# sethdford/csm-mlx

Hardware: AMD Instinct MI355X
Metric: audio frames/sec (24 kHz) csm_1b greedy, 10 s utterances, 1/2/4/8 GPU (higher is better)
Workload: dtype bf16; 1 GPU; csm_1b greedy generate(), 10 s utterances (125 frames) + Mimi decode; top_k=0, stream=False, context_segments=0, model=csm_1b (synthetic seed-0 weights), global_batch=1, per_gpu_batch=1, frames=125, mimi_decode=True, parallelism=dp1

## Files before the change

### csm-mlx_amd/csrc/bb_step.hip

```cpp
#include <type_traits>

#include "csm_kernels.h"
#include "handoff.h"

namespace {

using namespace handoff;

constexpr int NWG = BB_STEP_WGS, NT = BB_STEP_THREADS;
constexpr int D = 2048, F = 8192, HQ = 32, HKV = 8, HD = 64, NL = BB_STEP_LAYERS;
constexpr int QKV = (HQ + 2 * HKV) * HD;
constexpr int NATT = HQ;

constexpr int REP = 4;
constexpr size_t G_QKV = 0;
constexpr size_t G_ATT = G_QKV + 2 * QKV;
constexpr size_t G_X = G_ATT + 2 * REP * rs_of(D);
constexpr size_t G_PART = G_X + 2 * REP * rs_of(D);
constexpr size_t G_TOTAL = G_PART + (size_t)2 * NWG * D;

struct Lds {
  float x[D];
  float xn[D];
  float att[D];
  float red[8][NWG];
  float wsum[8][8];
  float sq[8];
  alignas(16) float hb[32];
  float2 rope[HD / 2];
  float q[HD], kn[HD], vn[HD];
  float am[8], al[8], ao[8][HD];
  float Ks[128][HD + 4], Vs[128][HD];
  alignas(16) float xq[D / 32][36];
  float xh[D / 32];
  alignas(16) float aq[D / 32][36];
  float ah[D / 32];
};

struct Ctx : HandoffCtx<BbStepArgs, Lds, REP> {
  __device__ void stamp(int slot) const {
    if (p.stamps && tid == 0 && slot < BB_STEP_STAMPS) p.stamps[(size_t)w * BB_STEP_STAMPS + slot] = __builtin_amdgcn_s_memrealtime();
  }
};

constexpr int PROBE_DELAY = 32;
constexpr int DELAY_E2 = PROBE_DELAY;

template <int GPT, int DELAY = PROBE_DELAY>
__device__ __forceinline__ void gather(Ctx& c, const u64* buf, int n, float* out) {
  const unsigned tag = c.tag();
  u64 g[GPT];
  __builtin_amdgcn_s_sleep(DELAY);
#pragma unroll
  for (int u = 0; u < GPT; ++u) {
    const int i = c.tid + u * NT;
    g[u] = i < n ? gload(buf + i) : ((u64)tag << 32);
  }
  for (unsigned spin = 0;; ++spin) {
    bool ok = true;
#pragma unroll
    for (int u = 0; u < GPT; ++u) ok &= (unsigned)(g[u] >> 32) == tag;
    if (ok || spin_fail(c, spin)) break;
    __builtin_amdgcn_s_sleep(1);
#pragma unroll
    for (int u = 0; u < GPT; ++u) {
      const int i = c.tid + u * NT;
      if (i < n && (unsigned)(g[u] >> 32) != tag) g[u] = gload(buf + i);
    }
  }
  c.stamp(c.e + 1);
#pragma unroll
  for (int u = 0; u < GPT; ++u) {
    const int i = c.tid + u * NT;
    if (i < n) out[i] = __uint_as_float((unsigned)g[u]);
  }
  __syncthreads();
}

__device__ __forceinline__ int el(const Ctx& c, int j) { return (j >> 1) * (D / 2) + 2 * c.tid + (j & 1); }
struct Nw { float v[D / NT]; };
__device__ __forceinline__ Nw nw_fetch(const Ctx& c, const float* nw) {
  Nw r;
#pragma unroll
  for (int j = 0; j < D / NT; ++j) r.v[j] = nw[el(c, j)];
  return r;
}
__device__ __forceinline__ void rms(Ctx& c, const Nw& nw, float* out) {
  if (c.wave == 0) {
    float s = 0.f;
#pragma unroll 8
    for (int k = c.lane; k < D; k += 64) s = fmaf(c.L.x[k], c.L.x[k], s);
    s = wave_sum(s);
    if (c.lane == 0) c.L.wsum[0][0] = s;
  }
  __syncthreads();
  const float r = rsqrtf(c.L.wsum[0][0] / (float)D + c.p.eps);
#pragma unroll
  for (int j = 0; j < D / NT; ++j) out[el(c, j)] = c.L.x[el(c, j)] * r * nw.v[j];
  __syncthreads();
}

__device__ __forceinline__ void gather_x(Ctx& c, const u64* buf, const Nw& nw) {
  constexpr int GPT = D / NT;
  const unsigned tag = c.tag();
  float sq = 0.f;
  const int poff[GPT / 2] = {2 * c.tid, D / 2 + 2 * c.tid};
  poll_pairs<GPT / 2, PROBE_DELAY, 1>(buf, 0x7fffffff, poff, tag, [&](unsigned spin) { return spin_fail(c, spin); },
                                      [&](const u32x4_t (&g)[GPT / 2]) {
#pragma unroll
    for (int h = 0; h < GPT / 2; ++h) {
      const float v0 = __uint_as_float(g[h].x), v1 = __uint_as_float(g[h].z);
      *reinterpret_cast<float2*>(&c.L.x[poff[h]]) = make_float2(v0, v1);
      *reinterpret_cast<float2*>(&c.L.xn[poff[h]]) = make_float2(v0 * nw.v[2 * h], v1 * nw.v[2 * h + 1]);
      sq = fmaf(v0, v0, sq);
      sq = fmaf(v1, v1, sq);
    }
  });
  c.stamp(c.e + 1);
  sq = wave_sum(sq);
  if (c.lane == 0) c.L.sq[c.wave] = sq;
  __syncthreads();
}
__device__ __forceinline__ float row_rs(const Ctx& c) {
  float s = c.L.sq[0];
#pragma unroll
  for (int w = 1; w < 8; ++w) s += c.L.sq[w];
  return rsqrtf(s / (float)D + c.p.eps);
}

struct WQ { u32x4_t a[6]; };
struct WO { u32x4_t a[4]; };
struct WMq { u32x4_t g[2][4]; u32x4_t d[4]; };

__device__ __forceinline__ void load_q(Ctx& c, int l, WQ& r) {
  const bf16_t* base = c.p.wqkv[l] + (size_t)(12 * c.w + 6 * (c.tid >> 8)) * D;
  const int v = (c.tid & 255) * 16;
#pragma unroll
  for (int i = 0; i < 6; ++i) r.a[i] = bload<2>(base, v, i * D * 2);
}
__device__ __forceinline__ void load_o(Ctx& c, int l, WO& r) {
  const bf16_t* base = c.p.wo[l] + (size_t)(8 * c.w + 4 * (c.tid >> 8)) * D;
  const int v = (c.tid & 255) * 16;
#pragma unroll
  for (int i = 0; i < 4; ++i) r.a[i] = bload<2>(base, v, i * D * 2);
}
__device__ __forceinline__ void load_mq(Ctx& c, int l, int Q, WMq& r) {
  const bf16_t* g = c.p.wgu[l] + (size_t)(64 * c.w + 16 * Q + 2 * c.wave) * D;
#pragma unroll
  for (int i = 0; i < 2; ++i)
#pragma unroll
    for (int j = 0; j < 4; ++j) r.g[i][j] = bload<2>(g, c.lane * 16, i * D * 2 + j * 64 * 16);
  const bf16_t* d = c.p.wdc[l] + (size_t)(4 * c.w + Q) * D * 8;
#pragma unroll
  for (int k = 0; k < 4; ++k)
    r.d[k] = bload<2>(d, c.tid * 16, k * NT * 8 * 2);
}

template <int R>
__device__ __forceinline__ void rows_reduce(Ctx& c, float (&s)[R]) {
#pragma unroll
  for (int i = 0; i < R; ++i) s[i] = wave_sum(s[i]);
  if (c.lane == 0) {
#pragma unroll
    for (int i = 0; i < R; ++i) c.L.wsum[c.wave][i] = s[i];
  }
  __syncthreads();
}
__device__ __forceinline__ float row_total(const Ctx& c, int h, int i) {
  return ((c.L.wsum[4 * h][i] + c.L.wsum[4 * h + 1][i]) + c.L.wsum[4 * h + 2][i]) + c.L.wsum[4 * h + 3][i];
}

__device__ __forceinline__ void phase_qkv(Ctx& c, int l, int pos, const WQ& W, bool sc) {
  float s[6];
  const float* xc = c.L.xn + 8 * (c.tid & 255);
#pragma unroll
  for (int i = 0; i < 6; ++i) s[i] = dot8(W.a[i], xc);
  rows_reduce<6>(c, s);
  if (c.tid < 6) {
    const int h = c.tid / 3, i0 = 2 * (c.tid % 3), n = 12 * c.w + 6 * h + i0;
    float a = row_total(c, h, i0), b = row_total(c, h, i0 + 1);
    if (sc) {
      const float rs = row_rs(c);
      a *= rs;
      b *= rs;
    }
    if (n < (HQ + HKV) * HD) {
      const float2 cs = c.L.rope[(n % HD) / 2];
      const float y0 = a * cs.x - b * cs.y, y1 = b * cs.x + a * cs.y;
      a = y0;
      b = y1;
    }
    u64* g = c.buf(G_QKV, QKV);
    gput(g + n, a, c.tag());
    gput(g + n + 1, b, c.tag());
    if (n >= HQ * HD) {
      const int nn = n < (HQ + HKV) * HD ? n - HQ * HD : n - (HQ + HKV) * HD;
      float* cache = n < (HQ + HKV) * HD ? c.p.kc[l] : c.p.vc[l];
      *reinterpret_cast<float2*>(cache + ((size_t)(nn / HD) * c.p.S_cap + pos) * HD + nn % HD) = make_float2(a, b);
    }
  }
}

struct KvPass { float4 kv[4], vv[4]; };

__device__ __forceinline__ void kv_pass_load(const Ctx& c, const float* K, const float* V, int pos, int k0, KvPass& kp) {
#pragma unroll
  for (int u = 0; u < 4; ++u) {
    const int idx = c.tid + NT * u, r = idx >> 4, c4 = idx & 15, j = k0 + r;
    const float4* ks = reinterpret_cast<const float4*>(j < pos ? K + (size_t)j * HD : c.L.kn);
    const float4* vs = reinterpret_cast<const float4*>(j < pos ? V + (size_t)j * HD : c.L.vn);
    kp.kv[u] = j <= pos ? ks[c4] : make_float4(0.f, 0.f, 0.f, 0.f);
    kp.vv[u] = j <= pos ? vs[c4] : make_float4(0.f, 0.f, 0.f, 0.f);
  }
}

__device__ __forceinline__ void attn_begin(Ctx& c, int l, int pos, KvPass& kp) {
  const int a = c.w, g = a / (HQ / HKV);
  {
    const u64* buf = c.p.gbuf + G_QKV + (size_t)((c.e - 1) & 1) * QKV;
    const unsigned tag = c.tag() - 1u;
    if (c.tid < 3 * HD) {
      const int part = c.tid / HD, d = c.tid % HD;
      const int idx = part == 0 ? a * HD + d : (part == 1 ? HQ * HD + g * HD + d : (HQ + HKV) * HD + g * HD + d);
      __builtin_amdgcn_s_sleep(PROBE_DELAY);
      u64 v = gload(buf + idx);
      for (unsigned spin = 0; (unsigned)(v >> 32) != tag; ++spin) {
        if (spin_fail(c, spin)) break;
        __builtin_amdgcn_s_sleep(1);
        v = gload(buf + idx);
      }
      const float f = __uint_as_float((unsigned)v);
      if (part == 0) c.L.q[d] = f * 0.125f;
      else if (part == 1) c.L.kn[d] = f;
      else c.L.vn[d] = f;
    }
    __syncthreads();
    c.stamp(c.e);
  }
// ... 15 lines not shown
      *reinterpret_cast<float4*>(&c.L.Ks[r][4 * c4]) = kp.kv[u];
      *reinterpret_cast<float4*>(&c.L.Vs[r][4 * c4]) = kp.vv[u];
    }
    __syncthreads();
    const int blk = c.wave - ((k0 >> 6) & 7);
    if (blk == 0 || blk == 1) {
      const int b0 = k0 + 64 * blk;
      if (b0 < n) {
        const int j = b0 + c.lane;
        const float4* kr = reinterpret_cast<const float4*>(c.L.Ks[64 * blk + c.lane]);
        const float4* q4 = reinterpret_cast<const float4*>(c.L.q);
        float d0 = 0.f, d1 = 0.f, d2 = 0.f, d3 = 0.f;
#pragma unroll
        for (int d4 = 0; d4 < HD / 4; ++d4) {
          const float4 qq = q4[d4], kk = kr[d4];
          d0 = fmaf(qq.x, kk.x, d0);
          d1 = fmaf(qq.y, kk.y, d1);
          d2 = fmaf(qq.z, kk.z, d2);
          d3 = fmaf(qq.w, kk.w, d3);
        }
        const float sc = j <= pos ? (d0 + d1) + (d2 + d3) : -INFINITY;
        const float m_new = fmaxf(m_run, wave_max(sc));
        const float alpha = m_run == -INFINITY ? 0.f : expf(m_run - m_new);
        const float pj = j <= pos ? expf(sc - m_new) : 0.f;
        l_run = l_run * alpha + wave_sum(pj);
        o *= alpha;
        const int pji = __float_as_int(pj);
#pragma unroll
        for (int u = 0; u < 64; ++u)
          o = fmaf(__int_as_float(__builtin_amdgcn_readlane(pji, u)), c.L.Vs[64 * blk + u][c.lane], o);
        m_run = m_new;
      }
    }
  }
  c.L.ao[c.wave][c.lane] = o;
  if (c.lane == 0) { c.L.am[c.wave] = m_run; c.L.al[c.wave] = l_run; }
  __syncthreads();
  if (c.wave < REP) {
    float M = -INFINITY;
#pragma unroll
    for (int v = 0; v < 8; ++v) M = fmaxf(M, c.L.am[v]);
    float Ls = 0.f, O = 0.f;
#pragma unroll
    for (int v = 0; v < 8; ++v) {
      const float wv = c.L.am[v] == -INFINITY ? 0.f : expf(c.L.am[v] - M);
      Ls = fmaf(c.L.al[v], wv, Ls);
      O = fmaf(c.L.ao[v][c.lane], wv, O);
    }
    c.put(G_ATT, D, a * HD + c.lane, O / Ls, c.wave);
  }
}

__device__ __forceinline__ void phase_o(Ctx& c, const WO& W) {
  float s[4];
  const float* xc = c.L.att + 8 * (c.tid & 255);
#pragma unroll
  for (int i = 0; i < 4; ++i) s[i] = dot8(W.a[i], xc);
  rows_reduce<4>(c, s);
  if (c.tid < 8 * REP) {
    const int q = c.tid / REP, h = q / 4, i = q % 4, n = 8 * c.w + q;
    c.put(G_X, D, n, c.L.x[n] + row_total(c, h, i), c.tid % REP);
  }
}

template <int Q>
__device__ __forceinline__ void phase_mq(Ctx& c, const WMq& m, float (&acc)[4], float rs) {
  float t[2];
#pragma unroll
  for (int i = 0; i < 2; ++i) {
    float s = dot8(m.g[i][0], c.L.xn + 8 * c.lane);
#pragma unroll
    for (int j = 1; j < 4; ++j) s += dot8(m.g[i][j], c.L.xn + 8 * (c.lane + 64 * j));
    t[i] = wave_sum(s);
  }
  if (c.lane == 0) c.L.hb[8 * Q + c.wave] = silu_f(rs * t[0]) * (rs * t[1]);
  __syncthreads();
#pragma unroll
  for (int k = 0; k < 4; ++k) {
    const float v = dot8(m.d[k], c.L.hb + 8 * Q);
    acc[k] = Q == 0 ? v : acc[k] + v;
  }
}

__device__ __forceinline__ void phase_reduce(Ctx& c) {
  const unsigned tag = c.tag();
  const u64* g = c.buf(G_PART, (size_t)NWG * D);
  const int v = c.tid >> 1, half = c.tid & 1;
  const int poff[2] = {v * D + 8 * c.w + 4 * half, v * D + 8 * c.w + 4 * half + 2};
  poll_pairs<2, PROBE_DELAY, 1>(g, 0x7fffffff, poff, tag, [&](unsigned spin) { return spin_fail(c, spin); },
                                [&](const u32x4_t (&q)[2]) {
#pragma unroll
    for (int h = 0; h < 2; ++h) {
      c.L.red[4 * half + 2 * h][v] = __uint_as_float(q[h].x);
      c.L.red[4 * half + 2 * h + 1][v] = __uint_as_float(q[h].z);
    }
  });
  c.stamp(c.e + 1);
  __syncthreads();
  ++c.e;
  {
    const float* r = c.L.red[c.wave];
    float s = ((r[4 * c.lane] + r[4 * c.lane + 1]) + r[4 * c.lane + 2]) + r[4 * c.lane + 3];
    s = wave_sum(s);
    if (c.lane < REP) {
      const int n = 8 * c.w + c.wave;
      c.put(G_X, D, n, c.L.x[n] + s, c.lane);
    }
  }
}

struct WQ4 { u32x4_t a[2]; unsigned s[2]; };
struct WO4 { u32x4_t a; unsigned s; };
struct WM4 { u32x4_t g[8]; unsigned gs[8]; u32x4_t d[4]; unsigned ds[4]; };
constexpr int RB = D / 2, SBR = D / 64 * 4;
constexpr int SB_QKV = QKV * RB, SB_O = D * RB, SB_GU = 2 * F * RB, SB_DN = D * F / 2;

__device__ __forceinline__ void load_q4(Ctx& c, int l, WQ4& r) {
  const char* W = reinterpret_cast<const char*>(c.p.wqkv[l]);
  const int r0 = 12 * c.w, va = c.wave * RB + c.lane * 16, vb = (8 + (c.wave & 3)) * RB + c.lane * 16;
  r.a[0] = bload<2>(W, va, r0 * RB);
  r.a[1] = bload<2>(W, vb, r0 * RB);
  const int sa = c.wave * SBR + (c.lane >> 1) * 4, sb = (8 + (c.wave & 3)) * SBR + (c.lane >> 1) * 4;
  r.s[0] = bload4(W, sa, SB_QKV + r0 * SBR);
  r.s[1] = bload4(W, sb, SB_QKV + r0 * SBR);
}
__device__ __forceinline__ void load_o4(Ctx& c, int l, WO4& r) {
  const char* W = reinterpret_cast<const char*>(c.p.wo[l]);
  r.a = bload<2>(W, c.wave * RB + c.lane * 16, 8 * c.w * RB);
  r.s = bload4(W, c.wave * SBR + (c.lane >> 1) * 4, SB_O + 8 * c.w * SBR);
}
__device__ __forceinline__ void load_m4(Ctx& c, int l, WM4& r) {
  const char* G = reinterpret_cast<const char*>(c.p.wgu[l]);
  const int r0 = 64 * c.w + 8 * c.wave;
#pragma unroll
  for (int i = 0; i < 8; ++i) {
    r.g[i] = bload<2>(G, 8 * c.wave * RB + c.lane * 16, (64 * c.w + i) * RB);
    r.gs[i] = bload4(G, 8 * c.wave * SBR + (c.lane >> 1) * 4, SB_GU + (64 * c.w + i) * SBR);
  }
  (void)r0;
  const char* Dn = reinterpret_cast<const char*>(c.p.wdc[l]);
#pragma unroll
  for (int k = 0; k < 4; ++k) {
    r.d[k] = bload<2>(Dn, c.tid * 16, (c.w * D + k * NT) * 16);
    r.ds[k] = bload4(Dn, c.tid * 4, SB_DN + ((c.w >> 1) * D + k * NT) * 4);
  }
}

__device__ __forceinline__ void half_group_sums(Ctx& c, const float (&pair)[2], float* out) {
#pragma unroll
  for (int h = 0; h < 2; ++h) {
    const float v = sum16(pair[h]);
    if ((c.tid & 15) == 0) out[(h * (D / 2) + 2 * c.tid) >> 5] = v;
  }
}
__device__ __forceinline__ void gather_x4(Ctx& c, const u64* buf, const Nw& nw) {
  const int poff[2] = {2 * c.tid, D / 2 + 2 * c.tid};
  float sq = 0.f, pr[2];
  poll_pairs<2, PROBE_DELAY, 1>(buf, 0x7fffffff, poff, c.tag(), [&](unsigned spin) { return spin_fail(c, spin); },
                                [&](const u32x4_t (&g)[2]) {
#pragma unroll
    for (int h = 0; h < 2; ++h) {
      const float v0 = __uint_as_float(g[h].x), v1 = __uint_as_float(g[h].z);
      const float a = v0 * nw.v[2 * h], b = v1 * nw.v[2 * h + 1];
      *reinterpret_cast<float2*>(&c.L.x[poff[h]]) = make_float2(v0, v1);
      *reinterpret_cast<float2*>(&c.L.xq[0][0] + q4p(poff[h])) = make_float2(a, b);
      sq = fmaf(v0, v0, sq);
// ... 89 lines not shown
  if (c.lane < 4) {
    const float gt = rs * (c.lane == 0 ? t[0] : (c.lane == 1 ? t[2] : (c.lane == 2 ? t[4] : t[6])));
    const float up = rs * (c.lane == 0 ? t[1] : (c.lane == 1 ? t[3] : (c.lane == 2 ? t[5] : t[7])));
    c.L.hb[4 * c.wave + c.lane] = silu_f(gt) * up;
  }
  __syncthreads();
  float hsum = 0.f;
#pragma unroll
  for (int j = 0; j < 32; j += 4) {
    const float4 v = *reinterpret_cast<const float4*>(&c.L.hb[j]);
    hsum += (v.x + v.y) + (v.z + v.w);
  }
#pragma unroll
  for (int k = 0; k < 4; ++k) acc[k] = q4dot32(W.d[k], c.L.hb, W.ds[k], hsum);
}

}

__global__ __launch_bounds__(NT, 1) void bb_step_q4_kernel(BbStepArgs p) {
  __shared__ __attribute__((aligned(16))) Lds L;
  Ctx c{{p, L, (int)blockIdx.x, (int)threadIdx.x, (int)(threadIdx.x & 63), (int)(threadIdx.x >> 6), 0u, 0}};
  c.tag0 = __hip_atomic_load(p.epoch, __ATOMIC_RELAXED, __HIP_MEMORY_SCOPE_AGENT) + 1u;
  c.stamp(0);
  const int pos = p.pos[0];
  WQ4 wq;
  WO4 wo;
  WM4 wm;
  load_q4(c, 0, wq);
  Nw nw1 = nw_fetch(c, p.n1[0]);
  for (int k = c.tid; k < D; k += NT) L.x[k] = p.x[k];
  if (c.tid < HD / 2) L.rope[c.tid] = reinterpret_cast<const float2*>(p.rope)[(size_t)pos * (HD / 2) + c.tid];
  __syncthreads();
  stage_x4(c, nw1);
  for (int l = 0; l < NL; ++l) {
    c.refresh();
    phase_qkv4(c, l, pos, wq);
    ++c.e;
    const bool attn_wg = c.w < NATT;
    if (!attn_wg) {
      load_o4(c, l, wo);
      load_m4(c, l, wm);
    }
    const Nw nw2 = nw_fetch(c, p.n2[l]);
    if (attn_wg) {
      KvPass kp;
      attn_begin(c, l, pos, kp);
      attn_rest(c, l, pos, kp);
      load_o4(c, l, wo);
      load_m4(c, l, wm);
    }
    if (attn_wg) gather_att4(c, c.rbuf(G_ATT, D));
    else gather_att4<DELAY_E2>(c, c.rbuf(G_ATT, D));
    ++c.e;
    c.refresh();
    phase_o4(c, wo);
    if (l + 1 < NL) load_q4(c, l + 1, wq);
    gather_x4(c, c.rbuf(G_X, D), nw2);
    const float rs2 = row_rs(c);
    ++c.e;
    c.refresh();
    float acc[4];
    phase_m4(c, wm, acc, rs2);
    {
      u64* g = c.buf(G_PART, (size_t)NWG * D) + (size_t)c.w * D;
#pragma unroll
      for (int k = 0; k < 4; ++k) gput(g + c.tid + NT * k, acc[k], c.tag());
    }
    nw1 = nw_fetch(c, l + 1 < NL ? p.n1[l + 1] : p.norm);
    c.refresh();
    phase_reduce(c);
    gather_x4(c, c.rbuf(G_X, D), nw1);
    ++c.e;
  }
  c.refresh();
  if (c.w == 0) {
    const float rs = row_rs(c);
    for (int k = c.tid; k < D; k += NT) p.h_last[k] = (&L.xq[0][0])[q4p(k)] * rs;
  }
  c.stamp(BB_STEP_STAMPS - 1);
  if (c.w == 0 && c.tid == 0) __hip_atomic_store(p.epoch, c.tag0 - 1u + (unsigned)c.e, __ATOMIC_RELAXED, __HIP_MEMORY_SCOPE_AGENT);
}

namespace {
}

__global__ __launch_bounds__(NT, 1) void bb_step_kernel(BbStepArgs p) {
  __shared__ __attribute__((aligned(16))) Lds L;
  Ctx c{{p, L, (int)blockIdx.x, (int)threadIdx.x, (int)(threadIdx.x & 63), (int)(threadIdx.x >> 6), 0u, 0}};
  c.tag0 = __hip_atomic_load(p.epoch, __ATOMIC_RELAXED, __HIP_MEMORY_SCOPE_AGENT) + 1u;
  c.stamp(0);
  const int pos = p.pos[0];
  WQ wq;
  WO wo;
  WMq mq[4];
  load_q(c, 0, wq);
  Nw nw1 = nw_fetch(c, p.n1[0]);
  for (int k = c.tid; k < D; k += NT) L.x[k] = p.x[k];
  if (c.tid < HD / 2) L.rope[c.tid] = reinterpret_cast<const float2*>(p.rope)[(size_t)pos * (HD / 2) + c.tid];
  __syncthreads();
  for (int l = 0; l < NL; ++l) {
    c.refresh();
    const bool fold1 = l > 0;
    if (!fold1) rms(c, nw1, L.xn);
    phase_qkv(c, l, pos, wq, fold1);
    ++c.e;
    const bool attn_wg = c.w < NATT;
    KvPass kp;
    load_o(c, l, wo);
    load_mq(c, l, 0, mq[0]);
    if (!attn_wg) {
      load_mq(c, l, 1, mq[1]);
      load_mq(c, l, 2, mq[2]);
    }
    const Nw nw2 = nw_fetch(c, p.n2[l]);
    if (attn_wg) {
      attn_begin(c, l, pos, kp);
      attn_rest(c, l, pos, kp);
      load_mq(c, l, 1, mq[1]);
    }
    if (attn_wg) gather<D / NT>(c, c.rbuf(G_ATT, D), D, L.att);
    else gather<D / NT, DELAY_E2>(c, c.rbuf(G_ATT, D), D, L.att);
    ++c.e;
    c.refresh();
    phase_o(c, wo);
    if (l + 1 < NL) load_q(c, l + 1, wq);
    gather_x(c, c.rbuf(G_X, D), nw2);
    const float rs2 = row_rs(c);
    ++c.e;
    c.refresh();
    float acc[4];
    phase_mq<0>(c, mq[0], acc, rs2);
    if (attn_wg) load_mq(c, l, 2, mq[2]);
    phase_mq<1>(c, mq[1], acc, rs2);
    load_mq(c, l, 3, mq[3]);
    phase_mq<2>(c, mq[2], acc, rs2);
    phase_mq<3>(c, mq[3], acc, rs2);
    {
      u64* g = c.buf(G_PART, (size_t)NWG * D) + (size_t)c.w * D;
#pragma unroll
      for (int k = 0; k < 4; ++k) gput(g + c.tid + NT * k, acc[k], c.tag());
    }
    nw1 = nw_fetch(c, l + 1 < NL ? p.n1[l + 1] : p.norm);
    c.refresh();
    phase_reduce(c);
    gather_x(c, c.rbuf(G_X, D), nw1);
    ++c.e;
  }
  c.refresh();
  if (c.w == 0) {
    const float rs = row_rs(c);
    for (int k = c.tid; k < D; k += NT) p.h_last[k] = L.xn[k] * rs;
  }
  c.stamp(BB_STEP_STAMPS - 1);
  if (c.w == 0 && c.tid == 0) __hip_atomic_store(p.epoch, c.tag0 - 1u + (unsigned)c.e, __ATOMIC_RELAXED, __HIP_MEMORY_SCOPE_AGENT);
}

size_t bb_step_gbuf_bytes() { return G_TOTAL * sizeof(u64); }

void launch_bb_step(const BbStepArgs& p, hipStream_t st, bool q4) {
  if (q4) hipLaunchKernelGGL(bb_step_q4_kernel, dim3(NWG), dim3(NT), 0, st, p);
  else hipLaunchKernelGGL(bb_step_kernel, dim3(NWG), dim3(NT), 0, st, p);
}

const void* bb_step_kernel_ptr(bool q4) {
  return q4 ? reinterpret_cast<const void*>(&bb_step_q4_kernel) : reinterpret_cast<const void*>(&bb_step_kernel);
}
```

### csm-mlx_amd/csrc/csm_engine_weights.hip

```cpp
#include "csm_engine.h"

namespace {

void alloc_stack(csm_engine* e, Stack& s, const csm_llama_dims& d, int S_cap, const char* prefix) {
  s.d = d;
  s.S_cap = S_cap;
  s.L.resize(d.n_layers);
  const size_t D = d.hidden, F = d.intermediate, hd = d.head_dim;
  for (int i = 0; i < d.n_layers; ++i) {
    LayerW& l = s.L[i];
    l.wqkv = e->alloc(e->wbytes(s.qkv_rows(), D));
    l.wo = e->alloc(e->wbytes(D, s.q_dim()));
    l.wgu = e->alloc(e->wbytes(2 * F, D));
    l.wd = e->alloc(e->wbytes(D, F));
    if (e->wdt == WDT_BF16 && wdc_chunk((int)D) && F % wdc_chunk((int)D) == 0) l.wdc = e->alloc(D * F * 2);
    l.n1 = (float*)e->alloc(D * 4);
    l.n2 = (float*)e->alloc(D * 4);
    const std::string p = std::string(prefix) + ".layers." + std::to_string(i);
    for (const char* n : {".self_attn.q_proj.weight", ".self_attn.k_proj.weight", ".self_attn.v_proj.weight",
                          ".self_attn.o_proj.weight", ".mlp.gate_proj.weight", ".mlp.up_proj.weight",
                          ".mlp.down_proj.weight", ".input_layernorm.weight", ".post_attention_layernorm.weight"})
      e->required.push_back(p + n);
  }
  s.norm = (float*)e->alloc(D * 4);
  s.rope = (float*)e->alloc((size_t)S_cap * hd * 4);
  e->required.push_back(std::string(prefix) + ".norm.weight");
}

}

void ensure_batch(csm_engine* e, int B) {
  if (B <= e->B_max && !e->batch_allocs.empty()) return;
  HIPCHK(hipDeviceSynchronize());
  for (void* p : e->batch_allocs) (void)hipFree(p);
  e->batch_allocs.clear();
  if (e->g_body) { (void)hipGraphExecDestroy(e->g_body); e->g_body = nullptr; }
  if (e->g_head) { (void)hipGraphExecDestroy(e->g_head); e->g_head = nullptr; }
  e->g_B = -1;
  e->B_max = std::max(B, e->B_max);
  const size_t Bm = e->B_max, D = e->D, Dd = e->Dd, K = e->K, Vp = e->Vpad;
  for (Stack* s : {&e->bb, &e->dec}) {
    const size_t kv = Bm * s->d.n_kv_heads * (size_t)s->S_cap * s->d.head_dim * 4;
    for (LayerW& l : s->L) {
      l.kc = (float*)e->balloc(kv);
      l.vc = (float*)e->balloc(kv);
    }
  }
  e->h_last = (float*)e->balloc(Bm * D * 4);
  e->c0_logits = (float*)e->balloc(Bm * Vp * 4);
  e->force = (int*)e->balloc(Bm * K * 4);
  e->force_ce = (float*)e->balloc(Bm * K * 4);
  e->ci_logits = (float*)e->balloc((K - 1) * Bm * Vp * 4);
  e->dx = (float*)e->balloc(2 * Bm * Dd * 4);
  e->din = (float*)e->balloc(2 * Bm * D * 4);
  e->dq = (float*)e->balloc(2 * Bm * e->dec.q_dim() * 4);
  e->datt = (float*)e->balloc(2 * Bm * e->dec.q_dim() * 4);
  e->dmlp = (float*)e->balloc(2 * Bm * (size_t)e->dec.d.intermediate * 4);
  e->codes = (int*)e->balloc(Bm * K * 4);
  e->hist = (int*)e->balloc((size_t)e->F_cap * Bm * K * 4);
  e->pos = (int*)e->balloc(Bm * 4);
  e->n_frames = (int*)e->balloc(Bm * 4);
  e->done = (uint8_t*)e->balloc(Bm);
  e->seeds = (uint64_t*)e->balloc(Bm * 8);
  e->part_stride = (int)(Vp / 2);
  e->part = (unsigned long long*)e->balloc(K * Bm * (size_t)e->part_stride * 8);
  for (Stack* s : {&e->bb, &e->dec}) {
    const int Dm = s->d.hidden, F = s->d.intermediate, rows = (s == &e->bb) ? std::max(e->M_cap, (int)Bm) : 2 * (int)Bm;
    gemm_reserve(e->ws, s->qkv_rows(), Dm, rows);
    gemm_reserve(e->ws, Dm, s->q_dim(), rows);
    gemm_reserve(e->ws, 2 * F, Dm, rows);
    gemm_reserve(e->ws, Dm, F, rows);
  }
  gemm_reserve(e->ws, (int)Dd, (int)D, 2 * (int)Bm);
  gemm_reserve(e->ws, (int)Vp, (int)D, (int)Bm);
  gemm_reserve(e->ws, (int)Vp, (int)Dd, (int)Bm);
  {
    const int xm = GEMM_XS_MAX_M, rows = std::min(2 * (int)Bm, xm);
    size_t bD = 0, bA = 0, bF = 0;
    for (Stack* s : {&e->bb, &e->dec}) {
      const int Dm = s->d.hidden, F = s->d.intermediate;
      bD = std::max(bD, xs::bytes(xm, Dm));
      bA = std::max(bA, xs::bytes(xm, s->q_dim()));
// ... 297 lines not shown
  }
  CSM_CATCH
}

int csm_engine_destroy(csm_engine* e) {
  CSM_TRY { delete e; }
  CSM_CATCH
}

int csm_set_rope_table(csm_engine* e, int which, const float* table, int n_pos, int head_dim) {
  CSM_TRY {
    Stack& s = which == 0 ? e->bb : e->dec;
    if (head_dim != s.d.head_dim || n_pos < s.S_cap) throw CsmError(CSM_ERR_ARG, "rope table shape mismatch");
    HIPCHK(hipSetDevice(e->dev));
    HIPCHK(hipMemcpy(s.rope, table, (size_t)s.S_cap * head_dim * 4, hipMemcpyHostToDevice));
  }
  CSM_CATCH
}

int csm_load_tensor(csm_engine* e, const char* cname, const void* host, int src_dtype, const int64_t* shape,
                    int ndim) {
  CSM_TRY {
    HIPCHK(hipSetDevice(e->dev));
    const std::string name(cname);
    std::vector<int64_t> shp(shape, shape + ndim);
    auto numel = [&]() { int64_t n = 1; for (auto s : shp) n *= s; return (size_t)n; };
    auto expect = [&](std::initializer_list<int64_t> want) {
      if (shp != std::vector<int64_t>(want)) throw CsmError(CSM_ERR_ARG, "shape mismatch for " + name);
    };
    if (name.rfind("decoder.layers.0.", 0) == 0) e->proj_tab_dirty = true;
    e->tiled_dirty = true;
    if (e->wdt == WDT_Q4 && load_q4(e, name, host, src_dtype, shp)) return CSM_OK;
    if (src_dtype == CSM_U32) throw CsmError(CSM_ERR_ARG, "packed int4 tensor " + name + " needs a CSM_Q4 engine");
    const size_t es = e->wsz;
    auto conv = [&](size_t n) { return convert_to(host, src_dtype, n, e->wdt); };
    auto conv_f32 = [&](size_t n) { return convert_to(host, src_dtype, n, WDT_F32); };

    for (int which = 0; which < 2; ++which) {
      Stack& s = which == 0 ? e->bb : e->dec;
      const std::string pre = which == 0 ? "backbone." : "decoder.";
      if (name.rfind(pre, 0) != 0) continue;
      const int D = s.d.hidden, F = s.d.intermediate, hd = s.d.head_dim;
      const int qd = s.q_dim(), kvd = s.d.n_kv_heads * hd;
      if (name == pre + "norm.weight") {
        expect({D});
        auto h = conv_f32(D);
        HIPCHK(hipMemcpy(s.norm, h.data(), D * 4, hipMemcpyHostToDevice));
        e->loaded.insert(name);
        return CSM_OK;
      }
      int li = -1;
      char tail[128] = {0};
      if (sscanf(name.c_str() + pre.size(), "layers.%d.%127s", &li, tail) != 2 || li < 0 || li >= s.d.n_layers)
        throw CsmError(CSM_ERR_ARG, "unknown tensor " + name);
      LayerW& l = s.L[li];
      const std::string t(tail);
      if (t == "self_attn.q_proj.weight") {
        expect({qd, D});
        auto h = conv(numel());
        HIPCHK(hipMemcpy(l.wqkv, h.data(), h.size(), hipMemcpyHostToDevice));
      } else if (t == "self_attn.k_proj.weight" || t == "self_attn.v_proj.weight") {
        expect({kvd, D});
        auto h = conv(numel());
        const size_t row0 = qd + (t[10] == 'k' ? 0 : kvd);
        HIPCHK(hipMemcpy((char*)l.wqkv + row0 * D * es, h.data(), h.size(), hipMemcpyHostToDevice));
      } else if (t == "self_attn.o_proj.weight") {
        expect({D, qd});
        auto h = conv(numel());
        HIPCHK(hipMemcpy(l.wo, h.data(), h.size(), hipMemcpyHostToDevice));
      } else if (t == "mlp.gate_proj.weight" || t == "mlp.up_proj.weight") {
        expect({F, D});
        auto h = conv(numel());
        const size_t off = (t[4] == 'g') ? 0 : 1;
        HIPCHK(hipMemcpy2D((char*)l.wgu + off * D * es, 2 * D * es, h.data(), D * es, D * es, F,
                           hipMemcpyHostToDevice));
      } else if (t == "mlp.down_proj.weight") {
        expect({D, F});
        auto h = conv(numel());
        HIPCHK(hipMemcpy(l.wd, h.data(), h.size(), hipMemcpyHostToDevice));
        if (l.wdc) {
          const int R = wdc_chunk(D);
          const uint16_t* src = reinterpret_cast<const uint16_t*>(h.data());
          std::vector<uint16_t> t2((size_t)D * F);
          for (int c = 0; c < F / R; ++c)
            for (int n = 0; n < D; ++n)
              memcpy(&t2[((size_t)c * D + n) * R], src + (size_t)n * F + (size_t)c * R, R * 2);
          HIPCHK(hipMemcpy(l.wdc, t2.data(), t2.size() * 2, hipMemcpyHostToDevice));
        }
      } else if (t == "input_layernorm.weight" || t == "post_attention_layernorm.weight") {
        expect({D});
        auto h = conv_f32(D);
        HIPCHK(hipMemcpy(t[0] == 'i' ? l.n1 : l.n2, h.data(), D * 4, hipMemcpyHostToDevice));
      } else {
        throw CsmError(CSM_ERR_ARG, "unknown tensor " + name);
      }
      e->loaded.insert(name);
      return CSM_OK;
    }
    const int64_t D = e->D, Dd = e->Dd, V = e->V, K = e->K, Vp = e->Vpad;
    if (name == "text_embeddings.weight") {
      expect({e->dims.n_text_vocab, D});
      auto h = conv(numel());
      HIPCHK(hipMemcpy(e->text_emb, h.data(), h.size(), hipMemcpyHostToDevice));
    } else if (name == "audio_embeddings.weight") {
      e->proj_tab_dirty = true;
      expect({V * K, D});
      auto h = conv(numel());
      HIPCHK(hipMemcpy(e->audio_emb, h.data(), h.size(), hipMemcpyHostToDevice));
    } else if (name == "projection.weight") {
      e->proj_tab_dirty = true;
      expect({Dd, D});
      auto h = conv(numel());
      HIPCHK(hipMemcpy(e->proj, h.data(), h.size(), hipMemcpyHostToDevice));
    } else if (name == "codebook0_head.weight") {
      expect({V, D});
      auto h = conv(numel());
      HIPCHK(hipMemcpy(e->c0_head, h.data(), h.size(), hipMemcpyHostToDevice));
    } else if (name == "audio_head") {
      expect({K - 1, Dd, V});
      auto f = conv_f32(numel());
      const float* src = reinterpret_cast<const float*>(f.data());
      std::vector<float> t((size_t)(K - 1) * Vp * Dd, 0.f);
      for (int64_t c = 0; c < K - 1; ++c)
        for (int64_t i = 0; i < Dd; ++i)
          for (int64_t v = 0; v < V; ++v) t[((size_t)c * Vp + v) * Dd + i] = src[((size_t)c * Dd + i) * V + v];
      auto h = convert_to(t.data(), CSM_F32, t.size(), e->head_wdt);
      HIPCHK(hipMemcpy(e->audio_head, h.data(), h.size(), hipMemcpyHostToDevice));
    } else {
      throw CsmError(CSM_ERR_ARG, "unknown tensor " + name);
    }
    e->loaded.insert(name);
  }
  CSM_CATCH
}

int csm_weights_ready(csm_engine* e) {
  CSM_TRY {
    for (const auto& n : e->required)
      if (!e->loaded.count(n)) throw CsmError(CSM_ERR_STATE, "missing weight " + n);
  }
  CSM_CATCH
}

static std::vector<std::pair<void*, size_t>> weight_buffers(csm_engine* e) {
  std::vector<std::pair<void*, size_t>> b;
  for (Stack* s : {&e->bb, &e->dec}) {
    const size_t D = s->d.hidden, F = s->d.intermediate;
    b.emplace_back(s->norm, D * 4);
    for (LayerW& l : s->L) {
      b.emplace_back(l.wqkv, e->wbytes(s->qkv_rows(), D));
      b.emplace_back(l.wo, e->wbytes(D, s->q_dim()));
      b.emplace_back(l.wgu, e->wbytes(2 * F, D));
      b.emplace_back(l.wd, e->wbytes(D, F));
      if (l.wdc) b.emplace_back(l.wdc, D * F * 2);
      b.emplace_back(l.n1, D * 4);
      b.emplace_back(l.n2, D * 4);
    }
  }
  const size_t D = e->D, Dd = e->Dd, V = e->V, K = e->K, Vp = e->Vpad;
  b.emplace_back(e->text_emb, e->wbytes(e->dims.n_text_vocab, D));
  b.emplace_back(e->audio_emb, e->wbytes(V * K, D));
  b.emplace_back(e->proj, e->wbytes(Dd, D));
  b.emplace_back(e->c0_head, e->wbytes(Vp, D));
  b.emplace_back(e->audio_head, (K - 1) * Vp * Dd * (e->head_wdt == WDT_F32 ? 4 : 2));
  return b;
}

int csm_weight_buffers(csm_engine* e, void** ptrs, uint64_t* bytes, int cap, int* n) {
  CSM_TRY {
// ... 70 lines not shown
```

### csm-mlx_amd/csrc/handoff.h

```cpp
#pragma once
#include "common.h"

namespace handoff {

typedef unsigned int u32x4_t __attribute__((ext_vector_type(4)));
typedef unsigned long long u64;

__device__ __forceinline__ u64 gload(const u64* p) {
  return __hip_atomic_load(p, __ATOMIC_RELAXED, __HIP_MEMORY_SCOPE_AGENT);
}
__device__ __forceinline__ void gput(u64* p, float v, unsigned tag) {
  __hip_atomic_store(p, ((u64)tag << 32) | __float_as_uint(v), __ATOMIC_RELAXED, __HIP_MEMORY_SCOPE_AGENT);
}
__device__ __forceinline__ void gput_u(u64* p, unsigned v, unsigned tag) {
  __hip_atomic_store(p, ((u64)tag << 32) | v, __ATOMIC_RELAXED, __HIP_MEMORY_SCOPE_AGENT);
}
__device__ __forceinline__ void sc1_store_f(float* p, float v) {
  __hip_atomic_store(p, v, __ATOMIC_RELAXED, __HIP_MEMORY_SCOPE_AGENT);
}

__device__ __forceinline__ u32x4_t sc1_load16(const void* base, int off, int bytes) {
  const __amdgpu_buffer_rsrc_t rs = __builtin_amdgcn_make_buffer_rsrc(const_cast<void*>(base), 0, bytes, 0x00020000);
  return __builtin_bit_cast(u32x4_t, __builtin_amdgcn_raw_buffer_load_b128(rs, off, 0, 16));
}
// ... 26 lines not shown
}
constexpr unsigned SPIN_LIMIT = 1u << 22;
template <typename C>
__device__ __forceinline__ bool spin_fail(const C& c, unsigned spin) { return spin_fail(c.p.err, SPIN_LIMIT, spin); }

__device__ __forceinline__ int opaque_tid() {
  int t;
  asm volatile("v_mov_b32 %0, %1" : "=v"(t) : "v"((int)threadIdx.x));
  return t;
}

__host__ __device__ constexpr size_t rs_of(size_t per) { return (per + 511) / 512 * 512 + 32; }
template <typename Args, typename Lds, int REP>
struct HandoffCtx {
  const Args& p;
  Lds& L;
  int w, tid, lane, wave;
  unsigned tag0;
  int e;
  __device__ void refresh() {
    tid = opaque_tid();
    lane = tid & 63;
    wave = tid >> 6;
  }
  __device__ unsigned tag() const { return tag0 + (unsigned)e; }
  __device__ u64* buf(size_t region, size_t per) const { return p.gbuf + region + (size_t)(e & 1) * per; }
  __device__ u64* rbuf(size_t region, size_t per, int r) const {
    return p.gbuf + region + ((size_t)(e & 1) * REP + (size_t)r) * rs_of(per);
  }
  __device__ u64* rbuf(size_t region, size_t per) const { return rbuf(region, per, w % REP); }
  __device__ void put(size_t region, size_t per, size_t i, float v, int r) const { gput(rbuf(region, per, r) + i, v, tag()); }
  __device__ void put_u(size_t region, size_t per, size_t i, unsigned v, int r) const {
    gput_u(rbuf(region, per, r) + i, v, tag());
  }
};

template <int GPT, int DELAY, int REPOLL, typename Fail, typename F>
__device__ __forceinline__ void poll_granules(const u64* base, const int (&off)[GPT], const bool (&val)[GPT], unsigned tag,
                                              Fail&& fail, F&& use) {
  auto cur = [&](const u64 (&x)[GPT]) {
    bool ok = true;
#pragma unroll
    for (int u = 0; u < GPT; ++u) ok &= !val[u] || (unsigned)(x[u] >> 32) == tag;
    return ok;
  };
  if constexpr (DELAY > 0) __builtin_amdgcn_s_sleep(DELAY);
  u64 g[GPT];
#pragma unroll
  for (int u = 0; u < GPT; ++u) g[u] = gload(base + (val[u] ? off[u] : 0));
  for (unsigned spin = 0; !cur(g) && !fail(spin); ++spin) {
    __builtin_amdgcn_s_sleep(REPOLL);
#pragma unroll
    for (int u = 0; u < GPT; ++u)
      if (val[u] && (unsigned)(g[u] >> 32) != tag) g[u] = gload(base + off[u]);
  }
  use(g);
}

template <int GPP, int DELAY, int REPOLL, typename Fail, typename F>
__device__ __forceinline__ void poll_pairs(const u64* base, int bytes, const int (&off)[GPP], unsigned tag, Fail&& fail, F&& use) {
  auto cur1 = [&](const u32x4_t& x) { return x.y == tag && x.w == tag; };
  if constexpr (DELAY > 0) __builtin_amdgcn_s_sleep(DELAY);
  u32x4_t g[GPP];
#pragma unroll
  for (int u = 0; u < GPP; ++u) g[u] = sc1_load16(base, off[u] * 8, bytes);
  for (unsigned spin = 0;; ++spin) {
    bool ok = true;
#pragma unroll
    for (int u = 0; u < GPP; ++u) ok &= cur1(g[u]);
    if (ok || fail(spin)) break;
    __builtin_amdgcn_s_sleep(REPOLL);
#pragma unroll
    for (int u = 0; u < GPP; ++u)
      if (!cur1(g[u])) g[u] = sc1_load16(base, off[u] * 8, bytes);
  }
  use(g);
}

template <int AUX = 0>
__device__ __forceinline__ unsigned bload4(const void* base, int voff, int soff) {
  const __amdgpu_buffer_rsrc_t rs = __builtin_amdgcn_make_buffer_rsrc(const_cast<void*>(base), 0, 0x7fffffff, 0x00020000);
  return __builtin_amdgcn_raw_buffer_load_b32(rs, voff, soff, AUX);
}
__device__ __forceinline__ float q4dot32(const u32x4_t w, const float* x, unsigned sb, float hs) {
  float d0 = 0.f, d1 = 0.f, d2 = 0.f, d3 = 0.f;
#pragma unroll
  for (int i = 0; i < 4; ++i) {
    const unsigned u = w[i], lo = u & 0x0F0F0F0Fu, hi = (u >> 4) & 0x0F0F0F0Fu;
    const float4 a = *reinterpret_cast<const float4*>(x + 8 * i), b = *reinterpret_cast<const float4*>(x + 8 * i + 4);
    d0 = fmaf((float)(lo & 0xFFu), a.x, d0);
    d1 = fmaf((float)(hi & 0xFFu), a.y, d1);
    d2 = fmaf((float)((lo >> 8) & 0xFFu), a.z, d2);
    d3 = fmaf((float)((hi >> 8) & 0xFFu), a.w, d3);
    d0 = fmaf((float)((lo >> 16) & 0xFFu), b.x, d0);
    d1 = fmaf((float)((hi >> 16) & 0xFFu), b.y, d1);
    d2 = fmaf((float)(lo >> 24), b.z, d2);
    d3 = fmaf((float)(hi >> 24), b.w, d3);
  }
  return fmaf(bf16_lo(sb), (d0 + d1) + (d2 + d3), bf16_hi(sb) * hs);
}
__device__ __forceinline__ float q4dot8(unsigned u, const float* x) {
  const unsigned lo = u & 0x0F0F0F0Fu, hi = (u >> 4) & 0x0F0F0F0Fu;
  const float4 a = *reinterpret_cast<const float4*>(x), b = *reinterpret_cast<const float4*>(x + 4);
  float s = (float)(lo & 0xFFu) * a.x;
  s = fmaf((float)(hi & 0xFFu), a.y, s);
  s = fmaf((float)((lo >> 8) & 0xFFu), a.z, s);
  s = fmaf((float)((hi >> 8) & 0xFFu), a.w, s);
  s = fmaf((float)((lo >> 16) & 0xFFu), b.x, s);
  s = fmaf((float)((hi >> 16) & 0xFFu), b.y, s);
  s = fmaf((float)(lo >> 24), b.z, s);
  s = fmaf((float)(hi >> 24), b.w, s);
  return s;
}
__device__ __forceinline__ int q4p(int k) { return (k >> 5) * 36 + (k & 31); }
__device__ __forceinline__ float2 half_sums(float v) {
  v += dpp_f<0x128>(v);
  v += dpp_f<0x124>(v);
  v += dpp_f<0x4E>(v);
  v += dpp_f<0xB1>(v);
  return make_float2(lane_f(v, 0) + lane_f(v, 16), lane_f(v, 32) + lane_f(v, 48));
}
__device__ __forceinline__ float sum16(float v) {
  v += __shfl_xor(v, 1, 64);
  v += __shfl_xor(v, 2, 64);
  v += __shfl_xor(v, 4, 64);
  v += __shfl_xor(v, 8, 64);
  return v;
}

}
```

Baseline: 419.7 audio frames/s.

## Rebalance MLP columns so attention workgroups own fewer FFN columns

The FFN columns are now split unevenly across the 256 workgroups. The 32 attention workgroups each get 4 columns and the other 224 get 36, instead of every workgroup owning 32. The kernel body is templated on whether a workgroup does attention, adds a tail path for column counts that are not a multiple of 8, and the host reorders the down-projection weights to match. The aim is to shorten the critical path, since attention workgroups otherwise finish their MLP share late and stall the cross-workgroup reduction. The cost is more code specialization and a weight layout tied to this particular split.

Result: no change. 421.1 audio frames/s (median of 2 runs) (+0.3%).

```diff
diff --git a/csm-mlx_amd/csrc/bb_split.h b/csm-mlx_amd/csrc/bb_split.h
--- /dev/null
+++ b/csm-mlx_amd/csrc/bb_split.h
@@ -0,0 +1,24 @@
+#pragma once
+
+constexpr int BB_F = 8192, BB_WGS = 256, BB_NATT = 32;
+constexpr int BB_CA = 4, BB_CN = 36;
+
+struct BbCols { int first, count; };
+constexpr BbCols bb_cols(int w) {
+  return w < BB_NATT ? BbCols{(BB_WGS - BB_NATT) * BB_CN + BB_CA * w, BB_CA} : BbCols{BB_CN * (w - BB_NATT), BB_CN};
+}
+
+constexpr bool bb_cols_partition() {
+  int owners[BB_F] = {};
+  for (int w = 0; w < BB_WGS; ++w) {
+    const BbCols c = bb_cols(w);
+    if (c.first < 0 || c.count < 0 || c.first + c.count > BB_F) return false;
+    for (int j = 0; j < c.count; ++j) ++owners[c.first + j];
+  }
+  for (int j = 0; j < BB_F; ++j)
+    if (owners[j] != 1) return false;
+  return true;
+}
+static_assert(bb_cols_partition(), "the workgroups' column slices must partition [0, F) with no gap or overlap");
+static_assert((BB_CA % 8 == 0 || BB_CA % 8 == 2 || BB_CA % 8 == 4) && (BB_CN % 8 == 0 || BB_CN % 8 == 2 || BB_CN % 8 == 4),
+              "a tail chunk row ([count % 8] bf16) is read as one 4-B or 8-B word");
diff --git a/csm-mlx_amd/csrc/bb_step.hip b/csm-mlx_amd/csrc/bb_step.hip
--- a/csm-mlx_amd/csrc/bb_step.hip
+++ b/csm-mlx_amd/csrc/bb_step.hip
@@ -1,5 +1,6 @@
 #include <type_traits>
 
+#include "bb_split.h"
 #include "csm_kernels.h"
 #include "handoff.h"
 
@@ -11,6 +12,7 @@
 constexpr int D = 2048, F = 8192, HQ = 32, HKV = 8, HD = 64, NL = BB_STEP_LAYERS;
 constexpr int QKV = (HQ + 2 * HKV) * HD;
 constexpr int NATT = HQ;
+static_assert(F == BB_F && NWG == BB_WGS && NATT == BB_NATT, "bb_split.h maps this kernel's grid");
 
 constexpr int REP = 4;
 constexpr size_t G_QKV = 0;
@@ -26,7 +28,7 @@
   float red[8][NWG];
   float wsum[8][8];
   float sq[8];
-  alignas(16) float hb[32];
+  alignas(16) float hb[40];
   float2 rope[HD / 2];
   float q[HD], kn[HD], vn[HD];
   float am[8], al[8], ao[8][HD];
@@ -42,6 +44,8 @@
     if (p.stamps && tid == 0 && slot < BB_STEP_STAMPS) p.stamps[(size_t)w * BB_STEP_STAMPS + slot] = __builtin_amdgcn_s_memrealtime();
   }
 };
+constexpr int STAMP_PUB = 81;
+static_assert(STAMP_PUB + 2 * BB_STEP_LAYERS < BB_STEP_STAMPS, "publish marks stay below the end-of-kernel slot");
 
 constexpr int PROBE_DELAY = 32;
 constexpr int DELAY_E2 = PROBE_DELAY;
@@ -131,6 +135,8 @@
 struct WQ { u32x4_t a[6]; };
 struct WO { u32x4_t a[4]; };
 struct WMq { u32x4_t g[2][4]; u32x4_t d[4]; };
+template <int T>
+struct WMt { u32x4_t g[2][4]; unsigned d[4][T / 2 > 0 ? T / 2 : 1]; };
 
 __device__ __forceinline__ void load_q(Ctx& c, int l, WQ& r) {
   const bf16_t* base = c.p.wqkv[l] + (size_t)(12 * c.w + 6 * (c.tid >> 8)) * D;
@@ -145,15 +151,37 @@
   for (int i = 0; i < 4; ++i) r.a[i] = bload<2>(base, v, i * D * 2);
 }
 __device__ __forceinline__ void load_mq(Ctx& c, int l, int Q, WMq& r) {
-  const bf16_t* g = c.p.wgu[l] + (size_t)(64 * c.w + 16 * Q + 2 * c.wave) * D;
+  const int col0 = bb_cols(c.w).first;
+  const bf16_t* g = c.p.wgu[l] + (size_t)(2 * (col0 + 8 * Q + c.wave)) * D;
 #pragma unroll
   for (int i = 0; i < 2; ++i)
 #pragma unroll
     for (int j = 0; j < 4; ++j) r.g[i][j] = bload<2>(g, c.lane * 16, i * D * 2 + j * 64 * 16);
-  const bf16_t* d = c.p.wdc[l] + (size_t)(4 * c.w + Q) * D * 8;
+  const bf16_t* d = c.p.wdc[l] + (size_t)D * col0 + (size_t)Q * D * 8;
 #pragma unroll
   for (int k = 0; k < 4; ++k)
     r.d[k] = bload<2>(d, c.tid * 16, k * NT * 8 * 2);
+}
+template <int T>
+__device__ __forceinline__ void load_mt(Ctx& c, int l, int NQ, WMt<T>& r) {
+  const int col0 = bb_cols(c.w).first + 8 * NQ;
+  const bf16_t* g = c.p.wgu[l] + (size_t)(2 * col0) * D;
+  const int v = c.wave < T ? 2 * c.wave * D * 2 + c.lane * 16 : 0;
+#pragma unroll
+  for (int i = 0; i < 2; ++i)
+#pragma unroll
+    for (int j = 0; j < 4; ++j) r.g[i][j] = bload<2>(g, v, i * D * 2 + j * 64 * 16);
+  const bf16_t* d = c.p.wdc[l] + (size_t)D * col0;
+#pragma unroll
+  for (int k = 0; k < 4; ++k) {
+    if constexpr (T == 2) {
+      r.d[k][0] = bload4<2>(d, c.tid * 4, k * NT * 4);
+    } else {
+      const u32x2_t x = bload8<2>(d, c.tid * 8, k * NT * 8);
+      r.d[k][0] = x.x;
+      r.d[k][1] = x.y;
+    }
+  }
 }
 
 template <int R>
@@ -335,6 +363,33 @@
   }
 }
 
+template <int T, int NQ>
+__device__ __forceinline__ void phase_mt(Ctx& c, const WMt<T>& m, float (&acc)[4], float rs) {
+  if (c.wave < T) {
+    float t[2];
+#pragma unroll
+    for (int i = 0; i < 2; ++i) {
+      float s = dot8(m.g[i][0], c.L.xn + 8 * c.lane);
+#pragma unroll
+      for (int j = 1; j < 4; ++j) s += dot8(m.g[i][j], c.L.xn + 8 * (c.lane + 64 * j));
+      t[i] = wave_sum(s);
+    }
+    if (c.lane == 0) c.L.hb[8 * NQ + c.wave] = silu_f(rs * t[0]) * (rs * t[1]);
+  }
+  __syncthreads();
+  const float* h = c.L.hb + 8 * NQ;
+#pragma unroll
+  for (int k = 0; k < 4; ++k) {
+    float v = bf16_lo(m.d[k][0]) * h[0];
+    v = fmaf(bf16_hi(m.d[k][0]), h[1], v);
+    if constexpr (T == 4) {
+      v = fmaf(bf16_lo(m.d[k][1]), h[2], v);
+      v = fmaf(bf16_hi(m.d[k][1]), h[3], v);
+    }
+    acc[k] = NQ == 0 ? v : acc[k] + v;
+  }
+}
+
 __device__ __forceinline__ void phase_reduce(Ctx& c) {
   const unsigned tag = c.tag();
   const u64* g = c.buf(G_PART, (size_t)NWG * D);
@@ -590,44 +645,42 @@
 }
 
 namespace {
-}
-
-__global__ __launch_bounds__(NT, 1) void bb_step_kernel(BbStepArgs p) {
-  __shared__ __attribute__((aligned(16))) Lds L;
-  Ctx c{{p, L, (int)blockIdx.x, (int)threadIdx.x, (int)(threadIdx.x & 63), (int)(threadIdx.x >> 6), 0u, 0}};
-  c.tag0 = __hip_atomic_load(p.epoch, __ATOMIC_RELAXED, __HIP_MEMORY_SCOPE_AGENT) + 1u;
-  c.stamp(0);
-  const int pos = p.pos[0];
-  WQ wq;
+
+template <bool ATT>
+__device__ __forceinline__ void bb_layers(Ctx& c, int pos, WQ& wq, Nw& nw1) {
+  constexpr int C = ATT ? BB_CA : BB_CN, NQ = C / 8, T = C % 8;
+  constexpr int HELD = ATT ? (NQ < 2 ? NQ : 2) : (NQ < 3 ? NQ : 3);
+  constexpr bool TAIL_EARLY = ATT && NQ <= 2;
+  static_assert(C > 0 && NQ <= 4, "a workgroup owns 1 to 32 + 7 columns");
+  const BbStepArgs& p = c.p;
+  Lds& L = c.L;
   WO wo;
   WMq mq[4];
-  load_q(c, 0, wq);
-  Nw nw1 = nw_fetch(c, p.n1[0]);
-  for (int k = c.tid; k < D; k += NT) L.x[k] = p.x[k];
-  if (c.tid < HD / 2) L.rope[c.tid] = reinterpret_cast<const float2*>(p.rope)[(size_t)pos * (HD / 2) + c.tid];
-  __syncthreads();
+  WMt<T> mt;
   for (int l = 0; l < NL; ++l) {
     c.refresh();
     const bool fold1 = l > 0;
     if (!fold1) rms(c, nw1, L.xn);
     phase_qkv(c, l, pos, wq, fold1);
     ++c.e;
-    const bool attn_wg = c.w < NATT;
-    KvPass kp;
-    load_o(c, l, wo);
-    load_mq(c, l, 0, mq[0]);
-    if (!attn_wg) {
-      load_mq(c, l, 1, mq[1]);
-      load_mq(c, l, 2, mq[2]);
+    if constexpr (!ATT || NQ > 0) {
+      load_o(c, l, wo);
+#pragma unroll
+      for (int q = 0; q < (ATT ? 1 : HELD); ++q) load_mq(c, l, q, mq[q]);
     }
     const Nw nw2 = nw_fetch(c, p.n2[l]);
-    if (attn_wg) {
+    if constexpr (ATT) {
+      KvPass kp;
       attn_begin(c, l, pos, kp);
       attn_rest(c, l, pos, kp);
-      load_mq(c, l, 1, mq[1]);
-    }
-    if (attn_wg) gather<D / NT>(c, c.rbuf(G_ATT, D), D, L.att);
-    else gather<D / NT, DELAY_E2>(c, c.rbuf(G_ATT, D), D, L.att);
+      c.stamp(STAMP_PUB + 2 * l + 1);
+      if constexpr (NQ == 0) load_o(c, l, wo);
+      if constexpr (HELD > 1) load_mq(c, l, 1, mq[1]);
+      if constexpr (T > 0 && TAIL_EARLY) load_mt<T>(c, l, NQ, mt);
+      gather<D / NT>(c, c.rbuf(G_ATT, D), D, L.att);
+    } else {
+      gather<D / NT, DELAY_E2>(c, c.rbuf(G_ATT, D), D, L.att);
+    }
     ++c.e;
     c.refresh();
     phase_o(c, wo);
@@ -637,23 +690,44 @@
     ++c.e;
     c.refresh();
     float acc[4];
-    phase_mq<0>(c, mq[0], acc, rs2);
-    if (attn_wg) load_mq(c, l, 2, mq[2]);
-    phase_mq<1>(c, mq[1], acc, rs2);
-    load_mq(c, l, 3, mq[3]);
-    phase_mq<2>(c, mq[2], acc, rs2);
-    phase_mq<3>(c, mq[3], acc, rs2);
+    if constexpr (NQ > 0) phase_mq<0>(c, mq[0], acc, rs2);
+    if constexpr (NQ > 2 && HELD < 3) load_mq(c, l, 2, mq[2]);
+    if constexpr (NQ > 1) phase_mq<1>(c, mq[1], acc, rs2);
+    if constexpr (NQ > 3) load_mq(c, l, 3, mq[3]);
+    if constexpr (T > 0 && !TAIL_EARLY) load_mt<T>(c, l, NQ, mt);
+    if constexpr (NQ > 2) phase_mq<2>(c, mq[2], acc, rs2);
+    if constexpr (NQ > 3) phase_mq<3>(c, mq[3], acc, rs2);
+    if constexpr (T > 0) phase_mt<T, NQ>(c, mt, acc, rs2);
     {
       u64* g = c.buf(G_PART, (size_t)NWG * D) + (size_t)c.w * D;
 #pragma unroll
       for (int k = 0; k < 4; ++k) gput(g + c.tid + NT * k, acc[k], c.tag());
     }
+    c.stamp(STAMP_PUB + 2 * l);
     nw1 = nw_fetch(c, l + 1 < NL ? p.n1[l + 1] : p.norm);
     c.refresh();
     phase_reduce(c);
     gather_x(c, c.rbuf(G_X, D), nw1);
     ++c.e;
   }
+}
+
+}
+
+__global__ __launch_bounds__(NT, 1) void bb_step_kernel(BbStepArgs p) {
+  __shared__ __attribute__((aligned(16))) Lds L;
+  Ctx c{{p, L, (int)blockIdx.x, (int)threadIdx.x, (int)(threadIdx.x & 63), (int)(threadIdx.x >> 6), 0u, 0}};
+  c.tag0 = __builtin_amdgcn_readfirstlane(__hip_atomic_load(p.epoch, __ATOMIC_RELAXED, __HIP_MEMORY_SCOPE_AGENT)) + 1u;
+  c.stamp(0);
+  const int pos = p.pos[0];
+  WQ wq;
+  load_q(c, 0, wq);
+  Nw nw1 = nw_fetch(c, p.n1[0]);
+  for (int k = c.tid; k < D; k += NT) L.x[k] = p.x[k];
+  if (c.tid < HD / 2) L.rope[c.tid] = reinterpret_cast<const float2*>(p.rope)[(size_t)pos * (HD / 2) + c.tid];
+  __syncthreads();
+  if (c.w < NATT) bb_layers<true>(c, pos, wq, nw1);
+  else bb_layers<false>(c, pos, wq, nw1);
   c.refresh();
   if (c.w == 0) {
     const float rs = row_rs(c);
diff --git a/csm-mlx_amd/csrc/csm_engine_weights.hip b/csm-mlx_amd/csrc/csm_engine_weights.hip
--- a/csm-mlx_amd/csrc/csm_engine_weights.hip
+++ b/csm-mlx_amd/csrc/csm_engine_weights.hip
@@ -1,3 +1,4 @@
+#include "bb_split.h"
 #include "csm_engine.h"
 
 namespace {
@@ -461,9 +462,18 @@
           const int R = wdc_chunk(D);
           const uint16_t* src = reinterpret_cast<const uint16_t*>(h.data());
           std::vector<uint16_t> t2((size_t)D * F);
-          for (int c = 0; c < F / R; ++c)
+          auto chunk = [&](int c0, int n_cols) {
             for (int n = 0; n < D; ++n)
-              memcpy(&t2[((size_t)c * D + n) * R], src + (size_t)n * F + (size_t)c * R, R * 2);
+              memcpy(&t2[(size_t)c0 * D + (size_t)n * n_cols], src + (size_t)n * F + c0, n_cols * 2);
+          };
+          if (which == 0 && D == 2048 && F == BB_F) {
+            for (int w = 0; w < BB_WGS; ++w) {
+              const BbCols cols = bb_cols(w);
+              for (int c0 = 0; c0 < cols.count; c0 += R) chunk(cols.first + c0, std::min(R, cols.count - c0));
+            }
+          } else {
+            for (int c = 0; c < F / R; ++c) chunk(c * R, R);
+          }
           HIPCHK(hipMemcpy(l.wdc, t2.data(), t2.size() * 2, hipMemcpyHostToDevice));
         }
       } else if (t == "input_layernorm.weight" || t == "post_attention_layernorm.weight") {
diff --git a/csm-mlx_amd/csrc/handoff.h b/csm-mlx_amd/csrc/handoff.h
--- a/csm-mlx_amd/csrc/handoff.h
+++ b/csm-mlx_amd/csrc/handoff.h
@@ -132,6 +132,12 @@
   const __amdgpu_buffer_rsrc_t rs = __builtin_amdgcn_make_buffer_rsrc(const_cast<void*>(base), 0, 0x7fffffff, 0x00020000);
   return __builtin_amdgcn_raw_buffer_load_b32(rs, voff, soff, AUX);
 }
+typedef unsigned int u32x2_t __attribute__((ext_vector_type(2)));
+template <int AUX = 0>
+__device__ __forceinline__ u32x2_t bload8(const void* base, int voff, int soff) {
+  const __amdgpu_buffer_rsrc_t rs = __builtin_amdgcn_make_buffer_rsrc(const_cast<void*>(base), 0, 0x7fffffff, 0x00020000);
+  return __builtin_bit_cast(u32x2_t, __builtin_amdgcn_raw_buffer_load_b64(rs, voff, soff, AUX));
+}
 __device__ __forceinline__ float q4dot32(const u32x4_t w, const float* x, unsigned sb, float hs) {
   float d0 = 0.f, d1 = 0.f, d2 = 0.f, d3 = 0.f;
 #pragma unroll
```
